# google/sbsim

Measured on AMD Instinct MI355X. Metric: zone-updates/sec (env-steps/sec x 9 zones) at batch=64k buildings per GPU, higher is better.
Workload: dtype f64

## Files before the change

sbsim_amd/csrc/runtime.hip:

```cpp
#include <hip/hip_runtime.h>

#include <algorithm>
#include <cmath>
#include <string>
#include <vector>

#include "sb_host.h"

using namespace sb;

namespace {

__global__ void k_reset(Dev a, double initial_temp, const double *temps, int first, int steps_since_reset, int temps_only) {
  const int lane = threadIdx.x & 63;
  const int wave = blockIdx.x * (blockDim.x >> 6) + (threadIdx.x >> 6);
  const int nwaves = gridDim.x * (blockDim.x >> 6);
  for (int b = wave; b < a.B; b += nwaves) {
    double s = 0.0, rlo = INFINITY, rhi = -INFINITY;
    if (a.reg) {
      double *T = a.temp + (size_t)b * a.state_doubles;
      const double *S0 = a.scal + (size_t)b * kNScal;
      const bool ring_uniform = S0[16] == S0[17];
      for (int g = lane; g < a.N; g += 64) {
        double v = temps ? temps[(size_t)b * a.N + g] : initial_temp;
// ... 206 lines not shown
}

__global__ void k_reset_jacobi(Dev a, float *grid, double initial_temp, const double *temps, int first, int steps_since_reset) {
  const int lane = threadIdx.x & 63;
  const int wave = blockIdx.x * (blockDim.x >> 6) + (threadIdx.x >> 6);
  const int nwaves = gridDim.x * (blockDim.x >> 6);
  for (int b = wave; b < a.B; b += nwaves) {
    double s = 0.0;
    for (int g = lane; g < a.N; g += 64) {
      const double v = temps ? temps[(size_t)b * a.N + g] : initial_temp;
      grid[(size_t)b * a.N + g] = (float)v;
      s += v;
    }
    s = wave_sum(s);
    for (int z = 0; z < a.Z; ++z) {
      double zs = 0.0;
      const int b0 = a.zone_off[z], b1 = a.zone_off[z + 1];
      for (int i = b0 + lane; i < b1; i += 64) zs += temps ? temps[(size_t)b * a.N + a.zone_cells_l[i]] : initial_temp;
      zs = wave_sum(zs);
      if (lane == 0) {
        const size_t o = (size_t)b * a.Z + z;
        a.zmean[o] = zs / (double)(b1 - b0);
        a.zair[o] = 0.0;
        a.damper[o] = 0.1;
        a.mode[o] &= kModeMask;
        a.qz[o] = 0.0;
      }
    }
    if (lane == 0) {
      double *S = a.scal + (size_t)b * kNScal;
      const double blr_sp = bparam(a, SB_BP_BLR_SETPOINT, b);
      S[0] = bparam(a, SB_BP_AHU_HEAT_SP, b); S[1] = bparam(a, SB_BP_AHU_COOL_SP, b); S[2] = 0.0; S[3] = 0.0;
      S[4] = blr_sp; S[5] = 0.0; S[6] = 0.0; S[7] = 0.0;
      S[8] = blr_sp; S[9] = 0.0; S[10] = 0.0;
      S[11] = s / (double)a.N;
      S[12] = S[13] = S[14] = S[15] = 0.0;
      S[16] = S[17] = 0.0;
      if (first) { S[18] = -1.0; S[19] = kAgeNone; }
      else if (!age_is_none(S[19])) S[19] -= (double)steps_since_reset;
    }
  }
}

__global__ void k_copy_temps_jacobi(const float *grid, size_t n, double *out) {
  for (size_t i = blockIdx.x * (size_t)blockDim.x + threadIdx.x; i < n; i += (size_t)gridDim.x * blockDim.x)
    out[i] = (double)grid[i];
}

constexpr int kRowsPerBlock = 16;
template <bool MAT, bool CLK>
__global__ void __launch_bounds__(16 * kRowsPerBlock) k_pre(Dev a, StepArgs s, int only) {
  if (blockIdx.x == 0 && threadIdx.x == 0) {
    *a.next_b = 0;
    if (a.redo_ctr) a.redo_ctr[0] = a.redo_ctr[1] = 0;
  }
  const int i = threadIdx.x & 15, r = threadIdx.x >> 4;
  if (only >= 0) {
    if (blockIdx.x == 0 && r == 0) pre_building<MAT, CLK>(a, s, only, i);
    return;
  }
  for (int b = blockIdx.x * kRowsPerBlock + r; b < a.B; b += gridDim.x * kRowsPerBlock) pre_building<MAT, CLK>(a, s, b, i);
}

void launch_pre(const sb_handle *h, const StepArgs &s, dim3 grid, hipStream_t stream, int only) {
  const dim3 block(16 * kRowsPerBlock);
  if (s.clk.rows) {
    if (h->d.ctab_b) hipLaunchKernelGGL((k_pre<true, true>), grid, block, 0, stream, h->d, s, only);
    else hipLaunchKernelGGL((k_pre<false, true>), grid, block, 0, stream, h->d, s, only);
  } else if (h->d.ctab_b) hipLaunchKernelGGL((k_pre<true, false>), grid, block, 0, stream, h->d, s, only);
  else hipLaunchKernelGGL((k_pre<false, false>), grid, block, 0, stream, h->d, s, only);
}

template <int KIND, bool CLK>
__global__ void __launch_bounds__(64) k_post(Dev a, StepArgs s, sb_reward_config rc, int only) {
  if (only >= 0) {
    if (blockIdx.x == 0 && threadIdx.x == 0) post_building<KIND, CLK>(a, s, rc, only);
    return;
  }
  for (int b = blockIdx.x * blockDim.x + threadIdx.x; b < a.B; b += gridDim.x * blockDim.x) post_building<KIND, CLK>(a, s, rc, b);
}

__global__ void __launch_bounds__(256) k_class_coef(const int4 *desc, const double *diff, const double *tab, int B, int ncls,
                                                    int M, double dt, double dx, double dx2, double zh, double *out) {
  const size_t n = (size_t)B * (ncls + 1);
  for (size_t i = blockIdx.x * (size_t)blockDim.x + threadIdx.x; i < n; i += (size_t)gridDim.x * blockDim.x) {
    const int b = (int)(i / (ncls + 1)), c = (int)(i - (size_t)b * (ncls + 1));
    double bn[4] = {0.0, 0.0, 0.0, 0.0}, ap = 0.0, gc = 0.0, sc = 0.0;
    if (c == ncls) {
      ap = 1.0;
    } else {
      const int4 e = desc[c];
      const double kk = tab[(size_t)e.x * B + b], cc = tab[(size_t)(M + e.x) * B + b], rr = tab[(size_t)(2 * M + e.x) * B + b];
      const double h_conv = tab[(size_t)3 * M * B + b];
      const int n_nb = e.y, present = e.z, half = e.w;
      if (n_nb <= 1) {
        gc = 1.0;
      } else if (n_nb == 2) {
        const double t0 = rr * dx2 * cc / dt / 2.0;
        const double den = 2.0 * kk + 2.0 * h_conv * dx + t0;
        for (int j = 0; j < 4; ++j)
          if (present >> j & 1) bn[j] = kk / den;
        ap = t0 / den; gc = 2.0 * h_conv * dx / den;
      } else if (n_nb == 3) {
        const double t0 = rr * dx2 / 2.0 * cc / dt;
        const double den = 2.0 * kk + h_conv * dx + t0;
        for (int j = 0; j < 4; ++j)
          if (present >> j & 1) bn[j] = kk * ((half >> j & 1) ? 0.5 : 1.0) / den;
// ... 136 lines not shown
  return SB_OK;
}

static int launch_observe(sb_handle *h, const sb_step_in &in, const double *t_amb_b, float *obs_dev, void *stream) {
  ClockView clk;
  SB_CHECK(clock_view(h, "sb_observe", &clk));
  SB_ON_DEVICE(h->device);
  const int blocks = std::max(1, std::min((h->d.B + 63) / 64, 4096));
  if (clk.rows) hipLaunchKernelGGL(k_observe<true>, dim3(blocks), dim3(64), 0, (hipStream_t)stream, h->d, clk, in, t_amb_b, obs_dev);
  else hipLaunchKernelGGL(k_observe<false>, dim3(blocks), dim3(64), 0, (hipStream_t)stream, h->d, clk, in, t_amb_b, obs_dev);
  SB_HIP(hipGetLastError());
  return SB_OK;
}

int sb_observe_occupancy(sb_handle *h, const float aux[SB_NUM_AUX], double t_amb, const double *t_amb_dev,
                         const float *num_occupants_dev, double occupancy_norm, float *obs_dev, void *stream) {
  if (!h || !aux || !obs_dev) return fail(SB_ERR_INVALID, "sb_observe: null argument");
  sb_step_in in{};
  in.t_amb_now = t_amb;
  in.num_occupants_dev = num_occupants_dev;
  in.occupancy_norm = occupancy_norm;
  std::copy_n(aux, SB_NUM_AUX, in.aux);
  return launch_observe(h, in, t_amb_dev, obs_dev, stream);
}

int sb_observe_step_in(sb_handle *h, const sb_step_in *in, float *obs_dev, void *stream) {
  if (!h || !in || !obs_dev) return fail(SB_ERR_INVALID, "sb_observe_step_in: null argument");
  return launch_observe(h, *in, nullptr, obs_dev, stream);
}

int sb_observe(sb_handle *h, const float aux[SB_NUM_AUX], double t_amb, const double *t_amb_dev,
               float *obs_dev, void *stream) {
  return sb_observe_occupancy(h, aux, t_amb, t_amb_dev, nullptr, 0.0, obs_dev, stream);
}

int sb_step_phases(sb_handle *h, const float *actions_dev, const sb_step_in *in, float *obs_dev,
                   float *reward_dev, float *info_dev, void *stream, int32_t phases) {
  if (!h || !in || !reward_dev) return fail(SB_ERR_INVALID, "sb_step: null argument");
  if (in->has_action && !actions_dev) return fail(SB_ERR_INVALID, "sb_step: has_action set but actions_dev is NULL");
  StepArgs s;
  s.actions = actions_dev; s.obs = obs_dev; s.reward = reward_dev; s.info = info_dev; s.in = *in;
  SB_CHECK(clock_view(h, "sb_step", &s.clk));
  SB_ON_DEVICE(h->device);
  const Dev &d = h->d;
  const int blocks = std::max(1, std::min((d.B + kRowsPerBlock - 1) / kRowsPerBlock, h->cus * 32));
  if (phases & SB_PHASE_PRE) {
    launch_pre(h, s, dim3(blocks), (hipStream_t)stream, -1);
    SB_HIP(hipGetLastError());
    h->counters_zeroed_on = stream;
  }
  if (phases & SB_PHASE_SWEEP) {
    if (h->counters_zeroed_on != stream) {
      SB_HIP(hipMemsetAsync(d.next_b, 0, sizeof(int), (hipStream_t)stream));
      if (d.redo_ctr) SB_HIP(hipMemsetAsync(d.redo_ctr, 0, 2 * sizeof(int), (hipStream_t)stream));
    }
    h->counters_zeroed_on = (void *)(uintptr_t)1;
    const int e = launch_sweep(h, (hipStream_t)stream);
    if (e != (int)hipSuccess)
      return fail(SB_ERR_HIP, std::string("sweep kernel launch: ") + hipGetErrorString((hipError_t)e));
  }
  if (phases & SB_PHASE_POST) {
    if (h->conv_attached) {
      const int rc = sb_launch_convection(h, (hipStream_t)stream);
      if (rc != SB_OK) return rc;
    }
    launch_post(h, s, dim3(std::max(1, std::min((d.B + 63) / 64, h->cus * 16))), (hipStream_t)stream, -1);
    ++h->steps_since_reset;
    SB_HIP(hipGetLastError());
  }
  return SB_OK;
}

int sb_step(sb_handle *h, const float *actions_dev, const sb_step_in *in, float *obs_dev,
            float *reward_dev, float *info_dev, void *stream) {
  return sb_step_phases(h, actions_dev, in, obs_dev, reward_dev, info_dev, stream,
                        SB_PHASE_PRE | SB_PHASE_SWEEP | SB_PHASE_POST);
}

int sb_get_temps(sb_handle *h, double *out_dev, void *stream) {
  if (!h || !out_dev) return fail(SB_ERR_INVALID, "sb_get_temps: null argument");
  SB_ON_DEVICE(h->device);
  if (h->kernel == SB_KERNEL_JACOBI)
    hipLaunchKernelGGL(k_copy_temps_jacobi, dim3(2048), dim3(256), 0, (hipStream_t)stream, h->jgrid.p,
                       (size_t)h->d.B * h->d.N, out_dev);
  else
    hipLaunchKernelGGL(k_copy_temps, dim3(2048), dim3(256), 0, (hipStream_t)stream, h->d, out_dev);
  SB_HIP(hipGetLastError());
  return SB_OK;
}

int sb_get_scalars(sb_handle *h, double *out_dev, void *stream) {
  if (!h || !out_dev) return fail(SB_ERR_INVALID, "sb_get_scalars: null argument");
  SB_ON_DEVICE(h->device);
  hipLaunchKernelGGL(k_copy_scalars, dim3(256), dim3(256), 0, (hipStream_t)stream, h->d, out_dev);
  SB_HIP(hipGetLastError());
  return SB_OK;
}

#define SB_COPY_OUT(name, src, count, type)                                                       \
  int name(sb_handle *h, type *out_dev, void *stream) {                                           \
    if (!h || !out_dev) return fail(SB_ERR_INVALID, #name ": null argument");                     \
    SB_ON_DEVICE(h->device);                                                              \
    SB_HIP(hipMemcpyAsync(out_dev, src, (size_t)(count) * sizeof(type), hipMemcpyDeviceToDevice,  \
                          (hipStream_t)stream));                                                  \
    return SB_OK;                                                                                 \
  }
SB_COPY_OUT(sb_get_zone_temps, h->d.zmean, (size_t)h->d.B *h->d.Z, double)
// ... 398 lines not shown
```

sbsim_amd/csrc/sb_device.h:

```cpp
#ifndef SBSIM_AMD_SB_DEVICE_H_
#define SBSIM_AMD_SB_DEVICE_H_

#include <hip/hip_runtime.h>

#include <stdint.h>

#include "sbsim_amd.h"

namespace sb {

constexpr double kCAir = 1006.0;
constexpr double kCWater = 4180.0;
constexpr double kRhoWater = 1000.0;
constexpr double kGravity = 9.8;
constexpr int kNScalOut = 16;
constexpr int kNScal = 20;
constexpr int kChunk = 8;
constexpr int kPad = 8;
constexpr double kAgeNone = -1e300;
__host__ __device__ inline bool age_is_none(double age) { return age < -1e200; }
constexpr int kModeMask = 0xff, kValveBit = 0x100;

struct Dev {
  int B, H, W, Z, N, Np, ncls, pitch, NL;
// ... 20 lines not shown
  int state_doubles;
  const uint8_t *tcls;
  const uint8_t *tcset;
  const double *tmulS;
  int tmul_doubles;
  const double *csetab;
  int ncset;
  int csetab_doubles;
  int two_sym, two_level;
  double *two_abuf;
  const int *zs_off;
  int tail_set_base, tail_pad_set;
  int RS;
  int AS;
  int ZRS;
  int Ws;
  int stream_ms;
  int n_ring;
  double n_ring_f64;
  int lw[4], l0[2], rowbase[2], nch[2];
  int lag;
  int nslots;
  float pred_haste;
  float pred_slack;
  int two_skip;
  float skip_kappa;
  int pred_first;
  int lds_reg_bytes;
  int wg_per_cu;
  int r_seam, r_A, r_zscr, r_xchg, r_zoff, r_zmode;
  int r_cmap;
  const unsigned long long *cmapS;
  const unsigned long long *amapS;
  const unsigned long long *zmapS;
  const int *cell_state;
  double *ring;
  double *temp;
  double *zmean;
  double *zair;
  double *damper;
  double *qz;
  int *mode;
  double *scal;
  struct Bld *bld;
  double *gtabg;
  double *zsum;
  double *gsum;
  int *nsw;
  int *next_b;
  int sweep_wgs;
  int *redo_ctr;
  int *redo_list;
  double *redo_scratch;
  int redo_mode;
  int roll_exact;
  int dbg_redo_mod;
  int roll_free;
  int O, col_ahu, col_blr, col_aux;
  const int *col_zone;
  const double *obs_mean, *obs_sigma;
  int n_src, n_hist, hist_normalize;
  const int *src_dest, *hist_col, *hist_off;
  const double *hist_bins;
  const int *act_kind, *act_zone;
  const double *act_lo, *act_hi;
  const int *zone_act;
  int n_damper_actions;
  long long *dbg;
  int dbg_timeline;
  sb_params p;
  const double *bp;
  const double *ctab_b;
  int off_wtab;
};

__host__ __device__ __forceinline__ double param_field(const sb_params &p, int k) {
  switch (k) {
    case SB_BP_VAV_MAX_AIR_FLOW: return p.vav_max_air_flow;
    case SB_BP_VAV_MAX_WATER_FLOW: return p.vav_max_water_flow;
    case SB_BP_AHU_RECIRC: return p.ahu_recirc;
    case SB_BP_AHU_HEAT_SP: return p.ahu_heat_sp;
    case SB_BP_AHU_COOL_SP: return p.ahu_cool_sp;
    case SB_BP_AHU_DP: return p.ahu_dp;
    case SB_BP_AHU_EFF: return p.ahu_eff;
    case SB_BP_AHU_MAX_FLOW: return p.ahu_max_flow;
    case SB_BP_BLR_SETPOINT: return p.blr_setpoint;
    case SB_BP_BLR_HEAD: return p.blr_head;
    case SB_BP_BLR_PUMP_EFF: return p.blr_pump_eff;
    case SB_BP_BLR_HEATING_RATE: return p.blr_heating_rate;
    case SB_BP_BLR_COOLING_RATE: return p.blr_cooling_rate;
    case SB_BP_BLR_CONV: return p.blr_conv;
    case SB_BP_BLR_LEN: return p.blr_len;
    case SB_BP_BLR_RADIUS: return p.blr_radius;
    case SB_BP_BLR_CAPACITY: return p.blr_capacity;
    case SB_BP_BLR_INS_K: return p.blr_ins_k;
    case SB_BP_BLR_INS_THICK: return p.blr_ins_thick;
    case SB_BP_COMFORT_LO: return p.comfort_lo;
    case SB_BP_COMFORT_HI: return p.comfort_hi;
    case SB_BP_ECO_LO: return p.eco_lo;
    case SB_BP_ECO_HI: return p.eco_hi;
    case SB_BP_MAX_PROD: return p.max_prod;
    case SB_BP_MIN_PROD: return p.min_prod;
    case SB_BP_MAX_ELEC: return p.max_elec;
    case SB_BP_MAX_GAS: return p.max_gas;
    case SB_BP_PROD_DELTA: return p.prod_delta;
    case SB_BP_PROD_STIFF: return p.prod_stiff;
    case SB_BP_W_PROD: return p.w_prod;
// ... 580 lines not shown
```

sbsim_amd/csrc/sbsim_hip.hip:

```cpp
#include <hip/hip_runtime.h>

#include <algorithm>
#include <cmath>
#include <cstdio>
#include <cstdlib>
#include <cstring>
#include <memory>
#include <string>
#include <vector>

#include "sb_host.h"

#ifndef SB_EXPERIMENTAL
namespace sb {
int launch_sweep_stream_ms(const Dev &, double *, double *, int, hipStream_t) { return (int)hipErrorNotSupported; }
int prepare_sweep_stream_ms(const Dev &, int) { return (int)hipErrorNotSupported; }
int sweep_stream_ms_sweeps() { return 1; }
int sweep_stream_ms_seam_doubles(int, int) { return 0; }
int sweep_stream_ms_xchg_doubles(int) { return 0; }
}
#endif

using namespace sb;

// ... 921 lines not shown
  Dev &d = h->d;
  for (int g = 0; g < d.N; ++g) h->h_state_index[g] = r.cell_state[g];
  d.pitch = d.W; d.NL = d.N; d.ts = r.ts;
  d.NR = r.NR; d.RS = r.RS; d.Ws = r.Ws; d.n_ring = r.n_ring; d.n_ring_f64 = (double)r.n_ring;
  d.T = r.T; d.state_doubles = r.state_doubles; d.AS = r.AS; d.ZRS = r.ZRS ? r.ZRS : (r.RS | 1);
  for (int w = 0; w < 2; ++w) { d.l0[w] = r.l0[w]; d.rowbase[w] = r.rowbase[w]; d.nch[w] = r.nch[w]; }
  for (int w = 0; w < 4; ++w) d.lw[w] = r.lw[w];
  d.lag = r.lag; d.nslots = r.nslots; d.nsteps = r.steps;
  d.lds_reg_bytes = r.lds_bytes; d.wg_per_cu = r.wg_per_cu;
  d.r_seam = r.r_seam; d.r_A = r.r_A; d.r_xchg = r.r_xchg;
  if (h->kernel == SB_KERNEL_ROLL) { d.r_cmap = r.r_cmap; d.lds_wave_doubles = r.wave_doubles; }
  d.pred_haste = k.pred_haste; d.pred_slack = k.pred_slack;
  if (h->kernel == SB_KERNEL_TWO_ROWS && !k.two_no_skip) {
    bool mono = true;
    for (int c = 0; c < plan->n_classes; ++c) {
      double sum = 0.0;
      for (int j = 0; j < 4; ++j) { mono = mono && plan->class_coef[c * 8 + j] >= 0.0; sum += plan->class_coef[c * 8 + j]; }
      mono = mono && sum <= 1.0;
    }
    d.two_skip = mono ? 1 : 0;
  }
  d.skip_kappa = k.skip_kappa;
  d.pred_first = h->kernel == SB_KERNEL_BAND ? 2 : 3;
  if (k.pred_first) d.pred_first = k.pred_first;
  SB_CHECK(upload(h->zone_cells_l, plan->zone_cells, (size_t)plan->zone_off[plan->Z]));
  SB_CHECK(upload(h->cmapS, r.cmapS.data(), r.cmapS.size()));
  SB_CHECK(upload(h->amapS, r.amapS.data(), r.amapS.size()));
  SB_CHECK(upload(h->zmapS, r.zmapS.data(), r.zmapS.size()));
  SB_CHECK(upload(h->cell_state, r.cell_state.data(), r.cell_state.size()));
  SB_CHECK(alloc_zero(h->ring, (size_t)d.B * std::max(r.n_ring, 1)));
  SB_CHECK(upload(h->tcls, r.tcls.data(), r.tcls.size()));
  SB_CHECK(upload(h->tcset, r.tcset.data(), r.tcset.size()));
  SB_CHECK(upload(h->csetab, r.csetab.data(), r.csetab.size()));
  SB_CHECK(upload(h->tmul, r.tmul.data(), r.tmul.size()));
  d.tmulS = h->tmul.p; d.tmul_doubles = (int)r.tmul.size();
  d.tcset = h->tcset.p; d.csetab = h->csetab.p; d.ncset = (int)r.csetab.size() / 4;
  d.csetab_doubles = (int)r.csetab.size();
  d.two_sym = r.two_sym; d.two_level = r.two_level; d.tail_set_base = r.tail_set_base;
  d.tail_pad_set = h->kernel == SB_KERNEL_TWO_ROWS ? r.tail_pad_set : (d.ncset - 1) * 32;
  if (!r.zs_off.empty()) {
    SB_CHECK(upload(h->zs_off, r.zs_off.data(), r.zs_off.size()));
    d.zs_off = h->zs_off.p;
  }
  SB_CHECK(alloc_zero(h->temp, (size_t)d.B * d.state_doubles));
  if (h->kernel == SB_KERNEL_STREAM) {
    SB_CHECK(alloc_zero(h->abuf, (size_t)h->info.workgroups * d.state_doubles));
    if (h->stream_variant != kStreamPlain) SB_CHECK(alloc_zero(h->ebuf, (size_t)h->info.workgroups * d.state_doubles));
  }
  if (h->kernel == SB_KERNEL_TWO_ROWS) {
    SB_CHECK(alloc_zero(h->abuf, (size_t)h->info.workgroups * (size_t)std::max(1, d.NR - sweep_two_lds_slots(d.NR, d.two_level)) * 128));
    d.two_abuf = h->abuf.p;
  }
  if (h->kernel == SB_KERNEL_ROLL) {
    SB_CHECK(alloc_zero(h->redo_ctr, 2));
    SB_CHECK(alloc_zero(h->redo_list, (size_t)d.B));
    SB_CHECK(alloc_zero(h->redo_scratch, (size_t)h->info.workgroups * h->info.waves_per_workgroup * d.state_doubles));
    d.redo_ctr = h->redo_ctr.p; d.redo_list = h->redo_list.p; d.redo_scratch = h->redo_scratch.p;
    d.roll_exact = k.roll_exact; d.dbg_redo_mod = k.force_redo; d.roll_free = k.roll_free;
  }
  d.tcls = h->tcls.p;
  d.cmapS = h->cmapS.p; d.amapS = h->amapS.p; d.zmapS = h->zmapS.p; d.cell_state = h->cell_state.p;
  d.ring = h->ring.p;
  return SB_OK;
}

int setup_lds(sb_handle *h, const sb_plan_desc *plan, const LdsPlan &q, const Knobs &k) {
  Dev &d = h->d;
  for (int g = 0; g < d.N; ++g) h->h_state_index[g] = kPad + g;
  d.pitch = q.pitch; d.NL = q.NL; d.S = q.S; d.S_magic = q.S_magic; d.nsteps = q.nsteps;
  d.nbands = q.nbands; d.fast = q.fast; d.ts = q.ts;
  if (k.force_generic) d.fast = 0;
  d.off_agtab = q.off_agtab; d.off_zscr = q.off_zscr; d.off_zmode = q.off_zmode; d.off_wtab = q.off_wtab;
  d.lds_wave_doubles = q.lds_wave_doubles;
  std::vector<int> zl((size_t)plan->zone_off[plan->Z]);
  for (size_t i = 0; i < zl.size(); ++i) {
    const int g = plan->zone_cells[i];
    zl[i] = (g / d.W) * d.pitch + g % d.W;
  }
  {
    std::vector<uint8_t> padded((size_t)d.N + 2 * kPad + 8, 0);
    std::memcpy(padded.data() + kPad, plan->cell_class, (size_t)d.N);
    SB_CHECK(upload(h->cls, padded.data(), padded.size()));
  }
  SB_CHECK(upload(h->zone_cells_l, zl.data(), zl.size()));
  {
    std::vector<uint16_t> idx;
    std::vector<int> bz;
    for (int z = 0; z < d.Z; ++z) {
      const int c0 = plan->zone_off[z], c1 = plan->zone_off[z + 1];
      std::vector<uint16_t> cells;
      for (int i = c0; i < c1; ++i) cells.push_back((uint16_t)zl[i]);
      while (cells.size() % 512) cells.push_back((uint16_t)d.NL);
      for (size_t b0 = 0; b0 < cells.size(); b0 += 512) {
        for (int l = 0; l < 64; ++l)
          for (int t = 0; t < 8; ++t) idx.push_back(cells[b0 + (size_t)t * 64 + l]);
        bz.push_back(z);
      }
    }
    if (idx.empty()) { idx.assign(512, (uint16_t)d.NL); bz.push_back(0); }
    d.n_zblocks = (int)bz.size();
    SB_CHECK(upload(h->zl16, (const uint4 *)idx.data(), idx.size() / 8));
    SB_CHECK(upload(h->zblk_zone, bz.data(), bz.size()));
  }
  {
    const int nch = (d.nsteps + kChunk - 1) / kChunk;
    const int nct = ((nch + 1) & ~1) + 6;
    std::vector<int4> sc((size_t)nct * 64);
// ... 323 lines not shown
```

sbsim_amd/csrc/step_roll.hip:

```cpp
#include "sweep_common.h"

namespace sb {
namespace {

using namespace sweep;

#ifndef SB_ONE_WAIT
#define SB_ONE_WAIT 1
#endif
constexpr int kWin = 63;
constexpr int kTS = 32;
constexpr int kSeamPad = 8;

constexpr int lds_slots(int NR) { return NR >= 72 ? 72 : ((NR / 2) % 2 ? NR : NR + 2); }
constexpr int a_stride(int NR) { return NR >= 72 ? 70 : ((NR / 2) % 2 ? NR : NR + 2); }
constexpr int kWaves = 4;
constexpr int tail_row(int NR) { return NR + 4; }

struct PairBuf {
  d2 ud0, lr0, ud1, lr1;
  d2 A;
  d2 sm;
};

// ... 217 lines not shown
    if constexpr (APASS && j0 < NR) pa.v[0] = ap.template fetch<j0 < NR ? j0 : 0>();
    if constexpr (APASS && j0 + 1 < NR) pa.v[1] = ap.template fetch<j0 + 1 < NR ? j0 + 1 : 0>();
    if constexpr (APASS && j0 + 2 < NR) pa.v[2] = ap.template fetch<j0 + 2 < NR ? j0 + 2 : 0>();
    __builtin_amdgcn_sched_barrier(0);
    if constexpr (S < kWin) step_ramp<NR, S, EXACT>(e, cur.ud0, cur.lr0, cur.A.x, acc, m0);
    else step<NR, S, EXACT, FREE>(e, bk, cur.ud0, cur.lr0, cur.A.x, cur.sm.x, acc);
    __builtin_amdgcn_sched_barrier(0);
    load_second<NR, N + 1>(nxt, x);
    __builtin_amdgcn_sched_barrier(0);
    if constexpr (S + 1 < kWin) step_ramp<NR, S + 1, EXACT>(e, cur.ud1, cur.lr1, cur.A.y, acc, m1);
    else step<NR, S + 1, EXACT, FREE>(e, bk, cur.ud1, cur.lr1, cur.A.y, cur.sm.y, acc);
    __builtin_amdgcn_sched_barrier(0);
    roll_pairs<NR, S + 2, S1, WRAP, EXACT, APASS, FREE>(e, bk, Areg, pb, x, acc, ap, pa);
  }
}

template <int NR, int J>
__device__ __forceinline__ void hand_over(double (&e)[NR], const double (&bk)[kWin], const unsigned long long (&zw)[NR / 8],
                                          double *tp, const double *np_, double *zrow) {
  static_assert(NR % 8 == 0, "whole zone words");
  if constexpr (J < NR) {
    if constexpr (J < kWin) e[J] = lanes_upto<J>() ? bk[J] : e[J];
    if constexpr (J + 1 < kWin) e[J + 1] = lanes_upto<J + 1>() ? bk[J + 1] : e[J + 1];
    const unsigned w = (J & 7) < 4 ? (unsigned)zw[J / 8] : (unsigned)(zw[J / 8] >> 32);
    const unsigned off0 = (w >> (8 * (J & 3))) & 0xffu, off1 = (w >> (8 * ((J + 1) & 3))) & 0xffu;
#ifndef SB_EXP_NOMEM
    __builtin_nontemporal_store(d2{e[J], e[J + 1]}, (d2 *)(tp + J * 64));
#endif
    __hip_atomic_fetch_add((double *)((char *)zrow + off0), e[J], __ATOMIC_RELAXED, __HIP_MEMORY_SCOPE_WORKGROUP);
    __hip_atomic_fetch_add((double *)((char *)zrow + off1), e[J + 1], __ATOMIC_RELAXED, __HIP_MEMORY_SCOPE_WORKGROUP);
#ifndef SB_EXP_NOMEM
    const d2 nv = __builtin_nontemporal_load((const d2 *)(np_ + J * 64));
    e[J] = nv.x;
    e[J + 1] = nv.y;
#endif
    if constexpr ((J & 7) == 6) __builtin_amdgcn_sched_barrier(0);
    hand_over<NR, J + 2>(e, bk, zw, tp, np_, zrow);
  }
}

template <int NR>
__device__ __forceinline__ void row63_to_tail(const double (&e)[NR], Acc &acc, int lane, double &U0, double &U1) {
  constexpr int last = (NR + kWin - 1) % NR;
  const double ul = wave_shift1<0x13c, false>(e[last], 0.0);
  double &sr = (NR - 1) % 2 == 0 ? acc.sre : acc.sro;
  sr = wave_shift1<0x138, true>(sr, ul);
  const int rev = (63 - lane) * 4;
  U0 = __hiloint2double(__builtin_amdgcn_ds_bpermute(rev, __double2hiint(acc.sre)),
                        __builtin_amdgcn_ds_bpermute(rev, __double2loint(acc.sre)));
  U1 = __hiloint2double(__builtin_amdgcn_ds_bpermute(rev, __double2hiint(acc.sro)),
                        __builtin_amdgcn_ds_bpermute(rev, __double2loint(acc.sro)));
}

extern __shared__ __attribute__((aligned(16))) double lds[];

template <int NR, bool EXACT>
__global__ void __launch_bounds__(64 * kWaves) __attribute__((amdgpu_waves_per_eu(1, 1))) k_sweep_roll(Dev a) {
  const int nB = a.redo_mode ? __builtin_amdgcn_readfirstlane(a.redo_ctr[0]) : a.B;
  if (nB == 0) return;
  const int lane = threadIdx.x & 63;
  const int wave = __builtin_amdgcn_readfirstlane((int)threadIdx.x >> 6);
  const int gw = (int)blockIdx.x * kWaves + wave;
  constexpr int kASlots = (NR + 7) / 8, kZSlots = NR / 8, kCW = NR / 8;
  static_assert((NR / 2) % kBufs == 0, "pair buffers rotate through a whole period: pair_buf() must not alias across the wrap");
  constexpr int kNL = lds_slots(NR), kAS = a_stride(NR), kNAR = NR - kNL > 0 ? NR - kNL : 2;

  double *tabc = lds;
  unsigned long long *ctab8 = (unsigned long long *)(lds + a.r_cmap);
  double *tmul = lds + a.r_cmap + kCW * 64;
  double *wl = tmul + a.tmul_doubles + (size_t)wave * a.lds_wave_doubles;
  double *tapg = wl;
  double *tE0 = wl + a.r_seam + 2;
  double *A = wl + a.r_A;
  for (int i = threadIdx.x; i < a.lds_reg_bytes / 8; i += blockDim.x) lds[i] = 0.0;
  __syncthreads();
  for (int i = threadIdx.x; i < 4 * kTS; i += blockDim.x) tabc[i] = i < 4 * a.ncset ? a.csetab[i] : 0.0;
  for (int i = threadIdx.x; i < kCW * 64; i += blockDim.x) ctab8[i] = a.cmapS[i];
  for (int i = threadIdx.x; i < a.tmul_doubles; i += blockDim.x) tmul[i] = a.tmulS[i];
  if (lane < kTS) tapg[lane] = lane <= a.ncls ? a.ctab[lane * 8 + 4] : 0.0;
  __syncthreads();

  const sb_params &p = a.p;
  const int R = lane;
  constexpr int RS = 64;
  if ((unsigned)(size_t)(__attribute__((address_space(3))) double *)tabc != 0u) __builtin_trap();
  Ctx<NR> x;
  x.Arow = A + (size_t)R * kAS;
  x.Aext = A + 64 * kAS + (size_t)R * (kNL - kAS);
  x.seam = tE0 - kWin;
  x.cw = ctab8 + lane;
  x.w = x.wn = 0;
#ifdef SB_EXP_NOCOEF
  x.kc = d2{0.2 + 1e-9 * opaque(lane), 0.2};
#endif
  const bool tactive = tail_col<NR>(lane, 0) >= 0;
  const int tc0 = tactive ? tail_col<NR>(lane, 0) : 0;
  const int tcw = tactive ? tc0 : -2;
  int tset[kTailMax], tcls8[kTailMax];
#pragma unroll
  for (int t = 0; t < kTailMax; ++t) {
    tset[t] = (a.ncset - 1) * 32 * 0x10001;
    tcls8[t] = (8 * a.ncls) | ((8 * a.ncls) << 8);
    if (t < a.T && tactive) {
      const int c0 = tc0, c1 = tc0 + 1;
      tset[t] = ((int)a.tcset[t * NR + c0] << 2) | ((int)a.tcset[t * NR + c1] << 18);
      tcls8[t] = (int)a.tcls[t * NR + c0] | ((int)a.tcls[t * NR + c1] << 8);
    }
  }
  const unsigned long long *amap = a.amapS + lane;
  const unsigned long long *zmap = a.zmapS + lane;

#ifdef SB_PHASE_STAMPS
#define SB_STAMP(i) do { if (a.dbg && gw == 0 && iter == 10 && lane == 0) a.dbg[i] = (long long)__builtin_readcyclecounter(); } while (0)
#else
#define SB_STAMP(i) do { } while (0)
#endif

  double e[NR];
  double nx_g = 0.0, nx_tail[kTailMax][2] = {{0.0, 0.0}, {0.0, 0.0}}, nx_tnow = 0.0, nx_lo = 0.0, nx_hi = 0.0;
#define SB_LOAD_AUX(bb)                                                                         \
  do {                                                                                          \
    nx_tnow = a.bld[(bb)].t_now;                                                                \
    nx_lo = a.scal[(size_t)(bb) * kNScal + 16];                                                 \
    nx_hi = a.scal[(size_t)(bb) * kNScal + 17];                                                 \
    nx_g = a.gtabg[(size_t)(bb) * kTS + (opaque(lane) & (kTS - 1))];  \
    const double *tt_ = a.temp + (size_t)(bb) * a.state_doubles + NR * 64;                      \
    _Pragma("unroll") for (int t = 0; t < kTailMax; ++t)                                        \
      _Pragma("unroll") for (int k = 0; k < 2; ++k)                                             \
        if (t < a.T) nx_tail[t][k] = tt_[t * NR + tc0 + k];                                     \
  } while (0)
  auto building = [&](int s) { return a.redo_mode ? __builtin_amdgcn_readfirstlane(a.redo_list[s]) : s; };
  const int b_first = gw < nB ? building(gw) : 0;
  if (gw < nB) {
    const double *tp_ = a.temp + (size_t)b_first * a.state_doubles;
#pragma unroll
    for (int j = 0; j < NR; j += 2) {
      const d2 v = __builtin_nontemporal_load((const d2 *)(tp_ + j * 64 + 2 * R));
      e[j] = v.x;
      e[j + 1] = v.y;
    }
    SB_LOAD_AUX(b_first);
  }
  unsigned long long amapw[kASlots];
#define SB_LOAD_AMAP(g0, g1)                                                                    \
  do {                                                                                          \
    const int o_ = opaque(0);                                                                   \
    _Pragma("unroll") for (int g = (g0); g < (g1); ++g) amapw[g] = amap[o_ + g * 64];           \
  } while (0)
  constexpr int kAHalf = kASlots / 2;
  SB_LOAD_AMAP(0, kASlots);
  int iter = 0;
  for (int s = gw, sn = 0, b = b_first, bn = 0; s < nB; s = sn, b = bn, ++iter) {
    int nb = 0;
    if (lane == 0) nb = atomicAdd(a.next_b, 1);
    SB_STAMP(0);
    x.wn = x.cw[0];
    __builtin_amdgcn_sched_barrier(0);
    const double t_now = nx_tnow;
    const double ring_d = a.n_ring > 0 ? fmax(fabs(t_now - nx_lo), fabs(t_now - nx_hi)) : 0.0;
    if (lane < kTS) tapg[kTS + opaque(lane)] = nx_g;
    double tv[kTailMax][2];
#pragma unroll
    for (int t = 0; t < kTailMax; ++t)
#pragma unroll
      for (int k = 0; k < 2; ++k) tv[t][k] = tactive ? nx_tail[t][k] : 0.0;
    *(d2 *)(tE0 + opaque(tcw)) = d2{tv[0][0], tv[0][1]};
    __builtin_amdgcn_wave_barrier();
    __builtin_amdgcn_sched_barrier(0);
    SB_STAMP(1);
    double At[kTailMax][2] = {{0.0, 0.0}, {0.0, 0.0}};
    if constexpr (!EXACT) {
      const double *pg[kTailMax][2];
#pragma unroll
      for (int t = 0; t < kTailMax; ++t)
#pragma unroll
        for (int k = 0; k < 2; ++k) pg[t][k] = (const double *)((const char *)tapg + ((opaque(tcls8[t]) >> (8 * k)) & 0xff));
      double tap[kTailMax][2], tg[kTailMax][2];
#pragma unroll
      for (int t = 0; t < kTailMax; ++t)
#pragma unroll
        for (int k = 0; k < 2; ++k) { tap[t][k] = pg[t][k][0]; tg[t][k] = pg[t][k][kTS]; }
#pragma unroll
      for (int t = 0; t < kTailMax; ++t)
#pragma unroll
        for (int k = 0; k < 2; ++k) At[t][k] = fma(tap[t][k], tv[t][k], tg[t][k]);
    } else {
#pragma unroll
      for (int t = 0; t < kTailMax; ++t)
#pragma unroll
        for (int k = 0; k < 2; ++k)
          if (t < a.T && tactive) {
            const int c8 = (opaque(tcls8[t]) >> (8 * k)) & 0xff;
            const double *pg = (const double *)((const char *)tapg + c8);
            At[t][k] = fma(pg[0], tv[t][k], pg[kTS]);
          }
    }

    double Areg[kNAR];
    Areg[0] = 0.0;
    const APass<NR, kNAR> ap{amapw, (unsigned)(size_t)(__attribute__((address_space(3))) double *)tapg, A + (size_t)R * kAS,
                             A + 64 * kAS + (size_t)R * (kNL - kAS), Areg};
    {
      static_assert(kA0 == 8 && kA0 + 3 * ((kWin - 3) / 2) >= NR, "the ramp-up's pairs but the last one reach the last slot");
      const d2 g0 = ap.template fetch<0>(), g1 = ap.template fetch<1>(), g2 = ap.template fetch<2>(), g3 = ap.template fetch<3>(),
               g4 = ap.template fetch<4>(), g5 = ap.template fetch<5>(), g6 = ap.template fetch<6>(), g7 = ap.template fetch<7>();
      __builtin_amdgcn_sched_barrier(0);
      ap.template put<0>(g0, e[0]); ap.template put<1>(g1, e[1]); ap.template put<2>(g2, e[2]); ap.template put<3>(g3, e[3]);
      ap.template put<4>(g4, e[4]); ap.template put<5>(g5, e[5]); ap.template put<6>(g6, e[6]); ap.template put<7>(g7, e[7]);
    }
    __builtin_amdgcn_wave_barrier();
    __builtin_amdgcn_sched_barrier(0);
    SB_STAMP(2);

    int n_sweeps = 0, converged = 0, redo = 0;
    double bk[kWin];
    {
      PairBuf pb[kBufs];
      Acc acc;
      acc.cur = 0.0; acc.neg = 0.0; acc.sg = lane == 0 ? (int)0x80000000 : 0;
      acc.tr = acc.fin = 0;
      acc.sre = acc.sro = 0.0;
      {
        const lds_d2 ct = step_set<NR, 0>(x);
        const d2 ud = ct[0], lr = ct[1];
        load_first<NR, 1, true>(pb[pair_buf(1)], x, Areg);
        load_second<NR, 2>(pb[pair_buf(1)], x);
        if constexpr (kDepth > 1) {
          load_first<NR, 3, true>(pb[pair_buf(3)], x, Areg);
          load_second<NR, 4>(pb[pair_buf(3)], x);
        }
        static_assert(kDepth <= 2, "initial fill of the pair buffers");
        step_ramp<NR, 0, EXACT>(e, ud, lr, x.Arow[1], acc, lanes_upto<0>());
      }
      __builtin_amdgcn_sched_barrier(0);
      roll_pairs<NR, 1, kWin, false, EXACT, true, false>(e, bk, Areg, pb, x, acc, ap);
#ifndef SB_STAMP_NEXT
      SB_STAMP(15);
#endif
#pragma nounroll
      for (;;) {
        __builtin_amdgcn_sched_barrier(0);
#ifdef SB_PHASE_STAMPS
#ifndef SB_STAMP_SWEEP
#define SB_STAMP_SWEEP 1
#endif
#define SB_STAMP2(i) do { if (a.dbg && gw == 0 && iter == 10 && sweep_idx == SB_STAMP_SWEEP && lane == 0) a.dbg[i] = (long long)__builtin_readcyclecounter(); } while (0)
        const int sweep_idx = n_sweeps;
#ifdef SB_STAMP_NEXT
        if (a.dbg && gw == 0 && iter == 10 && sweep_idx == SB_STAMP_SWEEP + 1 && lane == 0) a.dbg[15] = (long long)__builtin_readcyclecounter();
#endif
#else
#define SB_STAMP2(i) do { } while (0)
#endif
        if constexpr (!EXACT) {
          if (a.roll_free) {
            const int thr_top = __double2hiint(p.conv_threshold);
            int top = wave_max_i32(acc.tr);
            if (n_sweeps == 0) top = max(top, __double2hiint(ring_d));
#pragma nounroll
            while (top > thr_top && n_sweeps + 1 < p.iter_limit) {
              __builtin_amdgcn_sched_barrier(0);
              roll_pairs<NR, kWin, NR + kWin, true, false, false, true>(e, bk, Areg, pb, x, acc, ap);
              double F0, F1;
              row63_to_tail<NR>(e, acc, lane, F0, F1);
              tail_pass_static_values<NR>(a.T, tmul + opaque(tc0), tE0 + opaque(tcw), F0, F1, tv, tset, At);
              pb[pair_buf(kWin)].sm = *(const d2 *)(x.seam + kWin);
              if constexpr (kDepth > 1) pb[pair_buf(kWin + 2)].sm = *(const d2 *)(x.seam + kWin + 2);
              ++n_sweeps;
              acc.fin = 0;
              acc.tr = lanes_upto<62>() ? acc.tr : 0;
              top = wave_max_i32(acc.tr);
              __builtin_amdgcn_sched_barrier(0);
            }
          }
        }
        SB_STAMP2(10);
        roll_pairs<NR, kWin, NR + kWin, true, EXACT, false, false>(e, bk, Areg, pb, x, acc, ap);
        SB_STAMP2(11);
        double U0, U1;
        row63_to_tail<NR>(e, acc, lane, U0, U1);
        SB_STAMP2(12);
        const double dt_ = tail_pass_static<NR>(a.T, tmul + opaque(tc0), tE0 + opaque(tcw), U0, U1, tv, tset, At);

        SB_STAMP2(13);
        if constexpr (EXACT) {
          double md = wave_max(fmax(acc.cur, dt_));
          if (n_sweeps == 0) md = fmax(md, ring_d);
          ++n_sweeps;
          converged = md <= p.conv_threshold;
        } else {
          asm("v_max_f32 %0, %0, %1" : "+v"(acc.fin) : "v"(acc.tr));
          int m_hi = max(__builtin_amdgcn_readlane(acc.fin, 63), wave_max_i32(__double2hiint(dt_)));
          if (n_sweeps == 0) m_hi = max(m_hi, __double2hiint(ring_d));
          const int thr_hi = __double2hiint(p.conv_threshold);
          ++n_sweeps;
          acc.fin = 0;
          acc.tr = lanes_upto<62>() ? acc.tr : 0;
          const bool undecided = m_hi == thr_hi || (a.dbg_redo_mod > 0 && b % a.dbg_redo_mod == 0);
          if (m_hi <= thr_hi && undecided) { redo = 1; break; }
          converged = m_hi < thr_hi;
        }
        SB_STAMP2(14);
#ifdef SB_EXP_DESYNC
        if (n_sweeps >= 1 + (int)(((unsigned)b * 2654435761u >> 13) % 9u)) break;
#else
        if (converged || n_sweeps >= p.iter_limit) break;
#endif
        pb[pair_buf(kWin)].sm = *(const d2 *)(x.seam + kWin);
        if constexpr (kDepth > 1) pb[pair_buf(kWin + 2)].sm = *(const d2 *)(x.seam + kWin + 2);
        acc.cur = -acc.neg;
        acc.neg = 0.0;
        acc.sg = lane == 0 ? (int)0x80000000 : 0;
      }
    }
    __builtin_amdgcn_sched_barrier(0);
    SB_STAMP(3);
    sn = a.sweep_wgs + __builtin_amdgcn_readfirstlane(nb);
    bn = sn < nB ? building(sn) : 0;
    if (sn < nB) SB_LOAD_AUX(bn);
    SB_LOAD_AMAP(0, kAHalf);
    __builtin_amdgcn_sched_barrier(0);
    SB_STAMP(4);

    double *zs = A;
    const int ZRS = a.ZRS;
    {
      unsigned long long zw[kZSlots];
      const unsigned long long *zm = zmap + opaque(0);
#pragma unroll
      for (int g = 0; g < kZSlots; ++g) zw[g] = zm[g * 64];
      __builtin_amdgcn_sched_barrier(0);
      double *tp = redo ? a.redo_scratch + (size_t)gw * a.state_doubles : a.temp + (size_t)b * a.state_doubles;
      double *Ttail = tp + NR * 64;
      double *zrow = zs + (size_t)opaque(R) * ZRS;
      for (int z = 0; z <= a.Z; ++z) zrow[z] = 0.0;
      __builtin_amdgcn_wave_barrier();
#pragma unroll
      for (int t = 0; t < kTailMax; ++t)
        if (t < a.T && tactive) {
          *(d2 *)(Ttail + t * NR + tc0) = d2{tv[t][0], tv[t][1]};
          zrow[a.Z] += tv[t][0] + tv[t][1];
        }
      const double *np_ = a.temp + (size_t)(sn < nB ? bn : b) * a.state_doubles;
      static_assert(RS == 64, "hand_over: slot stride");
      hand_over<NR, 0>(e, bk, zw, tp + 2 * R, np_ + 2 * R, zrow);
    }
    __builtin_amdgcn_sched_barrier(0);
    SB_STAMP(5);
    SB_LOAD_AMAP(kAHalf, kASlots);
    __builtin_amdgcn_sched_barrier(0);
    SB_STAMP(6);
    __builtin_amdgcn_wave_barrier();
    SB_STAMP(7);

    {
      double gacc = 0.0;
      for (int zb = 0; zb <= a.Z; zb += 16) {
        const int zz = zb + (lane >> 2), g = lane & 3;
        const double *zr = zs + (size_t)g * ZRS + (zz <= a.Z ? zz : a.Z);
        double part[RS / 4];
#pragma unroll
        for (int k = 0; k < RS / 4; ++k) part[k] = zr[(size_t)4 * k * ZRS];
        double v = 0.0;
#pragma unroll
        for (int k = 0; k < RS / 4; ++k) v += part[k];
        if (zz > a.Z) v = 0.0;
        v += dpp_or_zero<0xB1, 0xf>(v);
        v += dpp_or_zero<0x4E, 0xf>(v);
        if (g == 0 && zz < a.Z && !redo) a.zsum[(size_t)b * a.Z + zz] = v;
        if (g == 0 && zz <= a.Z) gacc += v;
      }
      const double gsum = wave_sum(gacc);
      if (lane == 0 && !redo) {
        a.gsum[b] = gsum + a.n_ring_f64 * t_now;
        a.nsw[b] = n_sweeps | (converged << 16);
      }
      if (lane == 0 && redo) a.redo_list[atomicAdd(a.redo_ctr, 1)] = b;
      SB_STAMP(8);
#ifdef SB_PHASE_STAMPS
      if (a.dbg && gw == 0 && iter == 10 && lane == 0) a.dbg[9] = n_sweeps;
#endif
    }
  }
#undef SB_STAMP
#undef SB_LOAD_AUX
#undef SB_LOAD_AMAP
}

}

bool sweep_roll_supported(int NR) { return NR == 64 || NR == 72 || NR == 80 || NR == 88 || NR == 96; }
int sweep_roll_lds_slots(int NR) { return lds_slots(NR); }
int sweep_roll_a_stride(int NR) { return a_stride(NR); }
int sweep_roll_seam_doubles(int NR, int T) { (void)T; return tail_row(NR); }
int sweep_roll_waves() { return kWaves; }
int sweep_roll_tail_mul_doubles(int NR, int T) { return tail_mul_doubles(NR, T); }

int sweep_roll_redo_workgroups() { return 8; }

namespace {

template <int NR>
int prepare(const Dev &d) {
  const int e = (int)hipFuncSetAttribute((const void *)k_sweep_roll<NR, false>, hipFuncAttributeMaxDynamicSharedMemorySize,
                                         d.lds_reg_bytes);
  if (e != (int)hipSuccess) return e;
  return (int)hipFuncSetAttribute((const void *)k_sweep_roll<NR, true>, hipFuncAttributeMaxDynamicSharedMemorySize,
                                  d.lds_reg_bytes);
}

template <int NR>
int launch(const Dev &d, hipStream_t stream) {
  const dim3 grid((d.sweep_wgs + kWaves - 1) / kWaves), block(64 * kWaves);
  if (d.roll_exact) {
    hipLaunchKernelGGL((k_sweep_roll<NR, true>), grid, block, (size_t)d.lds_reg_bytes, stream, d);
    return (int)hipGetLastError();
  }
  hipLaunchKernelGGL((k_sweep_roll<NR, false>), grid, block, (size_t)d.lds_reg_bytes, stream, d);
  Dev r = d;
  r.redo_mode = 1;
  r.next_b = d.redo_ctr + 1;
  r.sweep_wgs = sweep_roll_redo_workgroups() * kWaves;
  hipLaunchKernelGGL((k_sweep_roll<NR, true>), dim3(sweep_roll_redo_workgroups()), block, (size_t)d.lds_reg_bytes, stream, r);
  return (int)hipGetLastError();
}

}

int prepare_sweep_roll(const Dev &d) {
  if (d.NR == 96) return prepare<96>(d);
  if (d.NR == 88) return prepare<88>(d);
  if (d.NR == 80) return prepare<80>(d);
  if (d.NR == 72) return prepare<72>(d);
  if (d.NR == 64) return prepare<64>(d);
  return (int)hipErrorInvalidValue;
}

int launch_sweep_roll(const Dev &d, hipStream_t stream) {
  if (d.NR == 96) return launch<96>(d, stream);
  if (d.NR == 88) return launch<88>(d, stream);
  if (d.NR == 80) return launch<80>(d, stream);
  if (d.NR == 72) return launch<72>(d, stream);
  if (d.NR == 64) return launch<64>(d, stream);
  return (int)hipErrorInvalidValue;
}

}
```

Before: 308.2 million.

## Fuse redo sweep into main roll kernel via in-kernel drain of redo list

Removes the second kernel launch that reprocessed undecided buildings with the exact path. Each wave now finishes its fast-path buildings, then drains the redo list itself by atomically claiming entries (stored as b+1, zeroed on claim). The redo work can then start while other waves are still on the fast path, instead of waiting for the whole kernel to end and then running on only 8 workgroups. Wave-wide max reductions in the convergence checks are replaced by ballots, and some address computations are restructured. The trade-offs are a larger fused kernel that may use more registers, and lock-free list claiming whose correctness depends on relaxed atomics and on redo entries being visible before waves drain.

```diff
diff --git a/sbsim_amd/csrc/runtime.hip b/sbsim_amd/csrc/runtime.hip
--- a/sbsim_amd/csrc/runtime.hip
+++ b/sbsim_amd/csrc/runtime.hip
@@ -282,7 +282,7 @@
 __global__ void __launch_bounds__(16 * kRowsPerBlock) k_pre(Dev a, StepArgs s, int only) {
   if (blockIdx.x == 0 && threadIdx.x == 0) {
     *a.next_b = 0;
-    if (a.redo_ctr) a.redo_ctr[0] = a.redo_ctr[1] = 0;
+    if (a.redo_ctr) *a.redo_ctr = 0;
   }
   const int i = threadIdx.x & 15, r = threadIdx.x >> 4;
   if (only >= 0) {
@@ -525,7 +525,7 @@
   if (phases & SB_PHASE_SWEEP) {
     if (h->counters_zeroed_on != stream) {
       SB_HIP(hipMemsetAsync(d.next_b, 0, sizeof(int), (hipStream_t)stream));
-      if (d.redo_ctr) SB_HIP(hipMemsetAsync(d.redo_ctr, 0, 2 * sizeof(int), (hipStream_t)stream));
+      if (d.redo_ctr) SB_HIP(hipMemsetAsync(d.redo_ctr, 0, sizeof(int), (hipStream_t)stream));
     }
     h->counters_zeroed_on = (void *)(uintptr_t)1;
     const int e = launch_sweep(h, (hipStream_t)stream);
diff --git a/sbsim_amd/csrc/sb_device.h b/sbsim_amd/csrc/sb_device.h
--- a/sbsim_amd/csrc/sb_device.h
+++ b/sbsim_amd/csrc/sb_device.h
@@ -96,7 +96,6 @@
   int *redo_ctr;
   int *redo_list;
   double *redo_scratch;
-  int redo_mode;
   int roll_exact;
   int dbg_redo_mod;
   int roll_free;
diff --git a/sbsim_amd/csrc/sbsim_hip.hip b/sbsim_amd/csrc/sbsim_hip.hip
--- a/sbsim_amd/csrc/sbsim_hip.hip
+++ b/sbsim_amd/csrc/sbsim_hip.hip
@@ -997,7 +997,7 @@
     d.two_abuf = h->abuf.p;
   }
   if (h->kernel == SB_KERNEL_ROLL) {
-    SB_CHECK(alloc_zero(h->redo_ctr, 2));
+    SB_CHECK(alloc_zero(h->redo_ctr, 1));
     SB_CHECK(alloc_zero(h->redo_list, (size_t)d.B));
     SB_CHECK(alloc_zero(h->redo_scratch, (size_t)h->info.workgroups * h->info.waves_per_workgroup * d.state_doubles));
     d.redo_ctr = h->redo_ctr.p; d.redo_list = h->redo_list.p; d.redo_scratch = h->redo_scratch.p;
diff --git a/sbsim_amd/csrc/step_roll.hip b/sbsim_amd/csrc/step_roll.hip
--- a/sbsim_amd/csrc/step_roll.hip
+++ b/sbsim_amd/csrc/step_roll.hip
@@ -293,43 +293,45 @@
                         __builtin_amdgcn_ds_bpermute(rev, __double2loint(acc.sro)));
 }
 
-extern __shared__ __attribute__((aligned(16))) double lds[];
+struct Wave {
+  int gw;
+  const unsigned long long *ctab8;
+  double *tmul;
+  double *wl;
+};
+
+__device__ __forceinline__ int take_redo(const Dev &a, int lane) {
+  const int n = __builtin_amdgcn_readfirstlane(__hip_atomic_load(a.redo_ctr, __ATOMIC_RELAXED, __HIP_MEMORY_SCOPE_AGENT));
+  for (int i0 = 0; i0 < n; i0 += 64) {
+    const int i = i0 + lane;
+    int v = 0;
+    if (i < n) v = __hip_atomic_load(a.redo_list + i, __ATOMIC_RELAXED, __HIP_MEMORY_SCOPE_AGENT);
+    for (unsigned long long m = __builtin_amdgcn_ballot_w64(v != 0); m; m &= m - 1) {
+      const int l = __builtin_ctzll(m);
+      int t = 0;
+      if (lane == l) t = __hip_atomic_exchange(a.redo_list + i, 0, __ATOMIC_RELAXED, __HIP_MEMORY_SCOPE_AGENT);
+      t = __builtin_amdgcn_readlane(t, l);
+      if (t) return t - 1;
+    }
+  }
+  return -1;
+}
 
 template <int NR, bool EXACT>
-__global__ void __launch_bounds__(64 * kWaves) __attribute__((amdgpu_waves_per_eu(1, 1))) k_sweep_roll(Dev a) {
-  const int nB = a.redo_mode ? __builtin_amdgcn_readfirstlane(a.redo_ctr[0]) : a.B;
-  if (nB == 0) return;
-  const int lane = threadIdx.x & 63;
-  const int wave = __builtin_amdgcn_readfirstlane((int)threadIdx.x >> 6);
-  const int gw = (int)blockIdx.x * kWaves + wave;
-  constexpr int kASlots = (NR + 7) / 8, kZSlots = NR / 8, kCW = NR / 8;
-  static_assert((NR / 2) % kBufs == 0, "pair buffers rotate through a whole period: pair_buf() must not alias across the wrap");
+__device__ __forceinline__ void run_buildings(const Dev &a, const Wave &w, const bool drain) {
+  const int nB = a.B;
+  const int lane = opaque((int)__lane_id()), gw = w.gw;
+  constexpr int kASlots = (NR + 7) / 8, kZSlots = NR / 8;
   constexpr int kNL = lds_slots(NR), kAS = a_stride(NR), kNAR = NR - kNL > 0 ? NR - kNL : 2;
-
-  double *tabc = lds;
-  unsigned long long *ctab8 = (unsigned long long *)(lds + a.r_cmap);
-  double *tmul = lds + a.r_cmap + kCW * 64;
-  double *wl = tmul + a.tmul_doubles + (size_t)wave * a.lds_wave_doubles;
-  double *tapg = wl;
-  double *tE0 = wl + a.r_seam + 2;
-  double *A = wl + a.r_A;
-  for (int i = threadIdx.x; i < a.lds_reg_bytes / 8; i += blockDim.x) lds[i] = 0.0;
-  __syncthreads();
-  for (int i = threadIdx.x; i < 4 * kTS; i += blockDim.x) tabc[i] = i < 4 * a.ncset ? a.csetab[i] : 0.0;
-  for (int i = threadIdx.x; i < kCW * 64; i += blockDim.x) ctab8[i] = a.cmapS[i];
-  for (int i = threadIdx.x; i < a.tmul_doubles; i += blockDim.x) tmul[i] = a.tmulS[i];
-  if (lane < kTS) tapg[lane] = lane <= a.ncls ? a.ctab[lane * 8 + 4] : 0.0;
-  __syncthreads();
-
-  const sb_params &p = a.p;
-  const int R = lane;
-  constexpr int RS = 64;
-  if ((unsigned)(size_t)(__attribute__((address_space(3))) double *)tabc != 0u) __builtin_trap();
+  double *const tmul = w.tmul;
+  double *const tapg = w.wl;
+  double *const tE0 = w.wl + a.r_seam + 2;
+  double *const A = w.wl + a.r_A;
   Ctx<NR> x;
-  x.Arow = A + (size_t)R * kAS;
-  x.Aext = A + 64 * kAS + (size_t)R * (kNL - kAS);
+  x.Arow = A + (size_t)lane * kAS;
+  x.Aext = A + 64 * kAS + (size_t)lane * (kNL - kAS);
   x.seam = tE0 - kWin;
-  x.cw = ctab8 + lane;
+  x.cw = w.ctab8 + lane;
   x.w = x.wn = 0;
 #ifdef SB_EXP_NOCOEF
   x.kc = d2{0.2 + 1e-9 * opaque(lane), 0.2};
@@ -348,8 +350,9 @@
       tcls8[t] = (int)a.tcls[t * NR + c0] | ((int)a.tcls[t * NR + c1] << 8);
     }
   }
-  const unsigned long long *amap = a.amapS + lane;
-  const unsigned long long *zmap = a.zmapS + lane;
+  const sb_params &p = a.p;
+  const int R = lane;
+  constexpr int RS = 64;
 
 #ifdef SB_PHASE_STAMPS
 #define SB_STAMP(i) do { if (a.dbg && gw == 0 && iter == 10 && lane == 0) a.dbg[i] = (long long)__builtin_readcyclecounter(); } while (0)
@@ -365,14 +368,27 @@
     nx_lo = a.scal[(size_t)(bb) * kNScal + 16];                                                 \
     nx_hi = a.scal[(size_t)(bb) * kNScal + 17];                                                 \
     nx_g = a.gtabg[(size_t)(bb) * kTS + (opaque(lane) & (kTS - 1))];  \
-    const double *tt_ = a.temp + (size_t)(bb) * a.state_doubles + NR * 64;                      \
+    const double *tt_ = a.temp + (size_t)(bb) * a.state_doubles + NR * 64 + opaque(tc0);  \
     _Pragma("unroll") for (int t = 0; t < kTailMax; ++t)                                        \
       _Pragma("unroll") for (int k = 0; k < 2; ++k)                                             \
-        if (t < a.T) nx_tail[t][k] = tt_[t * NR + tc0 + k];                                     \
+        if (t < a.T) nx_tail[t][k] = tt_[t * NR + k];                                           \
   } while (0)
-  auto building = [&](int s) { return a.redo_mode ? __builtin_amdgcn_readfirstlane(a.redo_list[s]) : s; };
-  const int b_first = gw < nB ? building(gw) : 0;
-  if (gw < nB) {
+  unsigned long long amapw[kASlots];
+#define SB_LOAD_AMAP(g0, g1)                                                                    \
+  do {                                                                                          \
+    const unsigned long long *am_ = a.amapS + opaque(lane);  \
+    _Pragma("unroll") for (int g = (g0); g < (g1); ++g) amapw[g] = am_[g * 64];                 \
+  } while (0)
+  constexpr int kAHalf = kASlots / 2;
+  for (;;) {
+  int b_first = gw;
+  if (drain) {
+    b_first = take_redo(a, lane);
+    if (b_first < 0) break;
+  } else if (gw >= nB) {
+    break;
+  }
+  {
     const double *tp_ = a.temp + (size_t)b_first * a.state_doubles;
 #pragma unroll
     for (int j = 0; j < NR; j += 2) {
@@ -382,18 +398,11 @@
     }
     SB_LOAD_AUX(b_first);
   }
-  unsigned long long amapw[kASlots];
-#define SB_LOAD_AMAP(g0, g1)                                                                    \
-  do {                                                                                          \
-    const int o_ = opaque(0);                                                                   \
-    _Pragma("unroll") for (int g = (g0); g < (g1); ++g) amapw[g] = amap[o_ + g * 64];           \
-  } while (0)
-  constexpr int kAHalf = kASlots / 2;
   SB_LOAD_AMAP(0, kASlots);
   int iter = 0;
-  for (int s = gw, sn = 0, b = b_first, bn = 0; s < nB; s = sn, b = bn, ++iter) {
+  for (int s = drain ? 0 : gw, sn = 0, b = b_first; s < nB; s = b = sn, ++iter) {
     int nb = 0;
-    if (lane == 0) nb = atomicAdd(a.next_b, 1);
+    if (lane == 0 && !drain) nb = atomicAdd(a.next_b, 1);
     SB_STAMP(0);
     x.wn = x.cw[0];
     __builtin_amdgcn_sched_barrier(0);
@@ -496,10 +505,10 @@
         if constexpr (!EXACT) {
           if (a.roll_free) {
             const int thr_top = __double2hiint(p.conv_threshold);
-            int top = wave_max_i32(acc.tr);
-            if (n_sweeps == 0) top = max(top, __double2hiint(ring_d));
+            bool top = __builtin_amdgcn_ballot_w64(acc.tr > thr_top) != 0;
+            if (n_sweeps == 0) top |= __double2hiint(ring_d) > thr_top;
 #pragma nounroll
-            while (top > thr_top && n_sweeps + 1 < p.iter_limit) {
+            while (top && n_sweeps + 1 < p.iter_limit) {
               __builtin_amdgcn_sched_barrier(0);
               roll_pairs<NR, kWin, NR + kWin, true, false, false, true>(e, bk, Areg, pb, x, acc, ap);
               double F0, F1;
@@ -510,7 +519,7 @@
               ++n_sweeps;
               acc.fin = 0;
               acc.tr = lanes_upto<62>() ? acc.tr : 0;
-              top = wave_max_i32(acc.tr);
+              top = __builtin_amdgcn_ballot_w64(acc.tr > thr_top) != 0;
               __builtin_amdgcn_sched_barrier(0);
             }
           }
@@ -531,15 +540,19 @@
           converged = md <= p.conv_threshold;
         } else {
           asm("v_max_f32 %0, %0, %1" : "+v"(acc.fin) : "v"(acc.tr));
-          int m_hi = max(__builtin_amdgcn_readlane(acc.fin, 63), wave_max_i32(__double2hiint(dt_)));
-          if (n_sweeps == 0) m_hi = max(m_hi, __double2hiint(ring_d));
+          const int cand = max(__double2hiint(dt_), lanes_upto<62>() ? 0 : acc.fin);
           const int thr_hi = __double2hiint(p.conv_threshold);
+          bool above = __builtin_amdgcn_ballot_w64(cand > thr_hi) != 0, equal = __builtin_amdgcn_ballot_w64(cand == thr_hi) != 0;
+          if (n_sweeps == 0) {
+            above |= __double2hiint(ring_d) > thr_hi;
+            equal |= __double2hiint(ring_d) == thr_hi;
+          }
           ++n_sweeps;
           acc.fin = 0;
           acc.tr = lanes_upto<62>() ? acc.tr : 0;
-          const bool undecided = m_hi == thr_hi || (a.dbg_redo_mod > 0 && b % a.dbg_redo_mod == 0);
-          if (m_hi <= thr_hi && undecided) { redo = 1; break; }
-          converged = m_hi < thr_hi;
+          const bool undecided = equal || (a.dbg_redo_mod > 0 && b % a.dbg_redo_mod == 0);
+          if (!above && undecided) { redo = 1; break; }
+          converged = !above && !equal;
         }
         SB_STAMP2(14);
 #ifdef SB_EXP_DESYNC
@@ -556,9 +569,8 @@
     }
     __builtin_amdgcn_sched_barrier(0);
     SB_STAMP(3);
-    sn = a.sweep_wgs + __builtin_amdgcn_readfirstlane(nb);
-    bn = sn < nB ? building(sn) : 0;
-    if (sn < nB) SB_LOAD_AUX(bn);
+    sn = drain ? nB : a.sweep_wgs + __builtin_amdgcn_readfirstlane(nb);
+    if (sn < nB) SB_LOAD_AUX(sn);
     SB_LOAD_AMAP(0, kAHalf);
     __builtin_amdgcn_sched_barrier(0);
     SB_STAMP(4);
@@ -567,7 +579,7 @@
     const int ZRS = a.ZRS;
     {
       unsigned long long zw[kZSlots];
-      const unsigned long long *zm = zmap + opaque(0);
+      const unsigned long long *zm = a.zmapS + opaque(lane);
 #pragma unroll
       for (int g = 0; g < kZSlots; ++g) zw[g] = zm[g * 64];
       __builtin_amdgcn_sched_barrier(0);
@@ -582,7 +594,7 @@
           *(d2 *)(Ttail + t * NR + tc0) = d2{tv[t][0], tv[t][1]};
           zrow[a.Z] += tv[t][0] + tv[t][1];
         }
-      const double *np_ = a.temp + (size_t)(sn < nB ? bn : b) * a.state_doubles;
+      const double *np_ = a.temp + (size_t)(sn < nB ? sn : b) * a.state_doubles;
       static_assert(RS == 64, "hand_over: slot stride");
       hand_over<NR, 0>(e, bk, zw, tp + 2 * R, np_ + 2 * R, zrow);
     }
@@ -616,16 +628,54 @@
         a.gsum[b] = gsum + a.n_ring_f64 * t_now;
         a.nsw[b] = n_sweeps | (converged << 16);
       }
-      if (lane == 0 && redo) a.redo_list[atomicAdd(a.redo_ctr, 1)] = b;
+      if constexpr (!EXACT) {
+        if (lane == 0 && redo)
+          __hip_atomic_store(a.redo_list + atomicAdd(a.redo_ctr, 1), b + 1, __ATOMIC_RELAXED, __HIP_MEMORY_SCOPE_AGENT);
+      }
       SB_STAMP(8);
 #ifdef SB_PHASE_STAMPS
       if (a.dbg && gw == 0 && iter == 10 && lane == 0) a.dbg[9] = n_sweeps;
 #endif
     }
   }
+  if (!drain) break;
+  }
 #undef SB_STAMP
 #undef SB_LOAD_AUX
 #undef SB_LOAD_AMAP
+}
+
+extern __shared__ __attribute__((aligned(16))) double lds[];
+
+template <int NR>
+__global__ void __launch_bounds__(64 * kWaves) __attribute__((amdgpu_waves_per_eu(1, 1))) k_sweep_roll(Dev a) {
+  if (a.B == 0) return;
+  const int lane = threadIdx.x & 63;
+  const int wave = __builtin_amdgcn_readfirstlane((int)threadIdx.x >> 6);
+  const int gw = (int)blockIdx.x * kWaves + wave;
+  constexpr int kCW = NR / 8;
+  static_assert((NR / 2) % kBufs == 0, "pair buffers rotate through a whole period: pair_buf() must not alias across the wrap");
+
+  double *tabc = lds;
+  unsigned long long *ctab8 = (unsigned long long *)(lds + a.r_cmap);
+  double *tmul = lds + a.r_cmap + kCW * 64;
+  double *wl = tmul + a.tmul_doubles + (size_t)wave * a.lds_wave_doubles;
+  double *tapg = wl;
+  for (int i = threadIdx.x; i < a.lds_reg_bytes / 8; i += blockDim.x) lds[i] = 0.0;
+  __syncthreads();
+  for (int i = threadIdx.x; i < 4 * kTS; i += blockDim.x) tabc[i] = i < 4 * a.ncset ? a.csetab[i] : 0.0;
+  for (int i = threadIdx.x; i < kCW * 64; i += blockDim.x) ctab8[i] = a.cmapS[i];
+  for (int i = threadIdx.x; i < a.tmul_doubles; i += blockDim.x) tmul[i] = a.tmulS[i];
+  if (lane < kTS) tapg[lane] = lane <= a.ncls ? a.ctab[lane * 8 + 4] : 0.0;
+  __syncthreads();
+
+  if ((unsigned)(size_t)(__attribute__((address_space(3))) double *)tabc != 0u) __builtin_trap();
+  const Wave w{gw, ctab8, tmul, wl};
+  const bool fast = !a.roll_exact;
+  if (fast) run_buildings<NR, false>(a, w, false);
+  auto *ka = __builtin_amdgcn_kernarg_segment_ptr();
+  asm volatile("" : "+s"(ka));
+  run_buildings<NR, true>(*(const Dev *)ka, w, fast);
 }
 
 }
@@ -637,32 +687,17 @@
 int sweep_roll_waves() { return kWaves; }
 int sweep_roll_tail_mul_doubles(int NR, int T) { return tail_mul_doubles(NR, T); }
 
-int sweep_roll_redo_workgroups() { return 8; }
-
 namespace {
 
 template <int NR>
 int prepare(const Dev &d) {
-  const int e = (int)hipFuncSetAttribute((const void *)k_sweep_roll<NR, false>, hipFuncAttributeMaxDynamicSharedMemorySize,
-                                         d.lds_reg_bytes);
-  if (e != (int)hipSuccess) return e;
-  return (int)hipFuncSetAttribute((const void *)k_sweep_roll<NR, true>, hipFuncAttributeMaxDynamicSharedMemorySize,
-                                  d.lds_reg_bytes);
+  return (int)hipFuncSetAttribute((const void *)k_sweep_roll<NR>, hipFuncAttributeMaxDynamicSharedMemorySize, d.lds_reg_bytes);
 }
 
 template <int NR>
 int launch(const Dev &d, hipStream_t stream) {
   const dim3 grid((d.sweep_wgs + kWaves - 1) / kWaves), block(64 * kWaves);
-  if (d.roll_exact) {
-    hipLaunchKernelGGL((k_sweep_roll<NR, true>), grid, block, (size_t)d.lds_reg_bytes, stream, d);
-    return (int)hipGetLastError();
-  }
-  hipLaunchKernelGGL((k_sweep_roll<NR, false>), grid, block, (size_t)d.lds_reg_bytes, stream, d);
-  Dev r = d;
-  r.redo_mode = 1;
-  r.next_b = d.redo_ctr + 1;
-  r.sweep_wgs = sweep_roll_redo_workgroups() * kWaves;
-  hipLaunchKernelGGL((k_sweep_roll<NR, true>), dim3(sweep_roll_redo_workgroups()), block, (size_t)d.lds_reg_bytes, stream, r);
+  hipLaunchKernelGGL((k_sweep_roll<NR>), grid, block, (size_t)d.lds_reg_bytes, stream, d);
   return (int)hipGetLastError();
 }
 
```

Result: no change. 309.1 million, median of 6 (+0.3%).
